# AberHu/TF-NAS

Measured on AMD Instinct MI355X. Metric: supernet search images/sec (w-step + alpha-step), higher is better.
Workload: dtype fp32

## Files before the change

### tf-nas_amd/csrc/gemm_core.h

```cpp
#pragma once
#include "tfnas_dev.h"

template <int NT>
struct GT {
    static constexpr int BM = 128, BK = 16, BN = 16 * NT;
    static constexpr int LDA = BM + 16;
    static constexpr int LDB = (BN % 32 == 16) ? BN : BN + 16;
    static constexpr int A_FLOATS = BK * LDA, B_FLOATS = BK * LDB;
    static constexpr int X3_FLOATS = 1584 * NT;
    static constexpr int LDS_FLOATS = 2 * (A_FLOATS + B_FLOATS) > X3_FLOATS ? 2 * (A_FLOATS + B_FLOATS) : X3_FLOATS;
    static constexpr int B_ITEMS = BN * 4;
    static constexpr int B_ITERS = (B_ITEMS + 255) / 256;
};

template <int NT>
__device__ __forceinline__ void acc_zero(f32x4 (&acc)[2][NT]) {
#pragma unroll
    for (int i = 0; i < 2; ++i)
#pragma unroll
        for (int j = 0; j < NT; ++j) acc[i][j] = zero4();
}

struct XfId {
    __device__ __forceinline__ f32x4 operator()(f32x4 v, int, int, int, int) const { return v; }
};

template <int NT, bool AK, bool BKC, bool BGUARD = true, class LA, class XA, class LB, class XB>
__device__ __forceinline__ void gemm_mainloop2(LA& la, XA& xa, LB& lb, XB& xb, int nchunks, f32x4 (&acc)[2][NT],
                                               float* lds) {
    using T = GT<NT>;
    using RA = decltype(la(0, 0, 0, 0));
    using RB = decltype(lb(0, 0, 0, 0));
    const int tid = threadIdx.x, lane = tid & 63, wrow = (tid >> 6) * 32;
    const int lr = lane & 15, lk = lane >> 4;
    RA ra[2];
    RB rb[T::B_ITERS];

#define TFNAS_A_IDX(i) const int idx = tid + 256 * (i), a0_ = AK ? (idx >> 2) : (idx >> 5), a1_ = AK ? (idx & 3) * 4 : (idx & 31) * 4
#define TFNAS_B_IDX(i)                                                      \
    const int idx = tid + 256 * (i), b0_ = BKC ? (idx >> 2) : idx / (T::BN / 4), \
              b1_ = BKC ? (idx & 3) * 4 : (idx % (T::BN / 4)) * 4
#define TFNAS_GLOAD(c)                                                                      \
    {                                                                                       \
        _Pragma("unroll") for (int i = 0; i < 2; ++i) {                                     \
            TFNAS_A_IDX(i);                                                                 \
            ra[i] = la((c), i, a0_, a1_);                                                      \
        }                                                                                   \
        _Pragma("unroll") for (int i = 0; i < T::B_ITERS; ++i) {                            \
            TFNAS_B_IDX(i);                                                                 \
            if (!BGUARD || idx < T::B_ITEMS) rb[i] = lb((c), i, b0_, b1_);                                \
        }                                                                                   \
    }
#define TFNAS_SSTORE(c, As, Bs)                                                             \
    {                                                                                       \
        _Pragma("unroll") for (int i = 0; i < 2; ++i) {                                     \
            TFNAS_A_IDX(i);                                                                 \
            const f32x4 v = xa(ra[i], (c), i, a0_, a1_);                                       \
            if (AK) {                                                                       \
                (As)[(a1_ + 0) * T::LDA + a0_] = v.x;                                       \
                (As)[(a1_ + 1) * T::LDA + a0_] = v.y;                                       \
                (As)[(a1_ + 2) * T::LDA + a0_] = v.z;                                       \
                (As)[(a1_ + 3) * T::LDA + a0_] = v.w;                                       \
            } else {                                                                        \
                st4(&(As)[a0_ * T::LDA + a1_], v);                                          \
            }                                                                               \
        }                                                                                   \
        _Pragma("unroll") for (int i = 0; i < T::B_ITERS; ++i) {                            \
            TFNAS_B_IDX(i);                                                                 \
            if (idx < T::B_ITEMS) {                                                         \
                const f32x4 v = xb(rb[i], (c), i, b0_, b1_);                                   \
                if (BKC) {                                                                  \
                    (Bs)[(b1_ + 0) * T::LDB + b0_] = v.x;                                   \
                    (Bs)[(b1_ + 1) * T::LDB + b0_] = v.y;                                   \
                    (Bs)[(b1_ + 2) * T::LDB + b0_] = v.z;                                   \
                    (Bs)[(b1_ + 3) * T::LDB + b0_] = v.w;                                   \
                } else {                                                                    \
                    st4(&(Bs)[b0_ * T::LDB + b1_], v);                                      \
                }                                                                           \
            }                                                                               \
        }                                                                                   \
    }

    float* As0 = lds;
    float* As1 = lds + T::A_FLOATS;
    float* Bs0 = lds + 2 * T::A_FLOATS;
    float* Bs1 = Bs0 + T::B_FLOATS;
#define TFNAS_MFMAS(As, Bs)                                                                 \
    _Pragma("unroll") for (int ks = 0; ks < 4; ++ks) {                                      \
        const int k = ks * 4 + lk;                                                          \
        const float a0 = (As)[k * T::LDA + wrow + lr];                                      \
        const float a1 = (As)[k * T::LDA + wrow + 16 + lr];                                 \
        _Pragma("unroll") for (int j = 0; j < NT; ++j) {                                    \
            const float b = (Bs)[k * T::LDB + 16 * j + lr];                                 \
            acc[0][j] = __builtin_amdgcn_mfma_f32_16x16x4f32(a0, b, acc[0][j], 0, 0, 0);    \
            acc[1][j] = __builtin_amdgcn_mfma_f32_16x16x4f32(a1, b, acc[1][j], 0, 0, 0);    \
        }                                                                                   \
    }

    if (nchunks > 0) {
        TFNAS_GLOAD(0);
        TFNAS_SSTORE(0, As0, Bs0);
    }
    __syncthreads();
    for (int c = 0; c < nchunks; ++c) {
        const bool more = (c + 1 < nchunks);
        if (more) TFNAS_GLOAD(c + 1);
        if (c & 1) { TFNAS_MFMAS(As1, Bs1); } else { TFNAS_MFMAS(As0, Bs0); }
        if (more) {
            if (c & 1) { TFNAS_SSTORE(c + 1, As0, Bs0); } else { TFNAS_SSTORE(c + 1, As1, Bs1); }
        }
        __syncthreads();
    }
#undef TFNAS_MFMAS
#undef TFNAS_GLOAD
#undef TFNAS_SSTORE
#undef TFNAS_A_IDX
#undef TFNAS_B_IDX
}

struct PreNone {
    __device__ __forceinline__ void operator()(int) const {}
};
template <int NT, bool BKC, class PRE, class LA, class XA, class LB, class XB>
__device__ __forceinline__ void gemm_mainloop_adirect(PRE& pre, LA& la, XA& xa, LB& lb, XB& xb, int nchunks,
                                                      f32x4 (&acc)[2][NT], float* lds) {
    using T = GT<NT>;
    using RA = decltype(la(0, 0, 0));
    using RB = decltype(lb(0, 0, 0));
    const int tid = threadIdx.x, lane = tid & 63;
    const int lr = lane & 15, lk = lane >> 4;
    RA ra[2];
    RB rb[T::B_ITERS];
    f32x4 cur[2];

#define TFNAS_B_IDX(i)                                                      \
    const int idx = tid + 256 * (i), b0_ = BKC ? (idx >> 2) : idx / (T::BN / 4), \
              b1_ = BKC ? (idx & 3) * 4 : (idx % (T::BN / 4)) * 4
#define TFNAS_GLOAD(c)                                                                      \
    {                                                                                       \
        pre(c);                                                                             \
        _Pragma("unroll") for (int i = 0; i < 2; ++i) ra[i] = la((c), i, 4 * lk);           \
        _Pragma("unroll") for (int i = 0; i < T::B_ITERS; ++i) {                            \
            TFNAS_B_IDX(i);                                                                 \
            if (idx < T::B_ITEMS) rb[i] = lb((c), b0_, b1_);                                \
        }                                                                                   \
    }
#define TFNAS_SSTORE(c, Bs)                                                                 \
    {                                                                                       \
        _Pragma("unroll") for (int i = 0; i < 2; ++i) cur[i] = xa(ra[i], (c), i, 4 * lk);   \
        _Pragma("unroll") for (int i = 0; i < T::B_ITERS; ++i) {                            \
            TFNAS_B_IDX(i);                                                                 \
            if (idx < T::B_ITEMS) {                                                         \
                const f32x4 v = xb(rb[i], (c), b0_, b1_);                                   \
                if (BKC) {                          \
                    const int r0_ = b1_ >> 2;                                               \
                    (Bs)[(r0_ + 0) * T::LDB + b0_] = v.x;                                   \
                    (Bs)[(r0_ + 4) * T::LDB + b0_] = v.y;                                   \
                    (Bs)[(r0_ + 8) * T::LDB + b0_] = v.z;                                   \
                    (Bs)[(r0_ + 12) * T::LDB + b0_] = v.w;                                  \
                } else {                                                                    \
                    st4(&(Bs)[((b0_ & 3) * 4 + (b0_ >> 2)) * T::LDB + b1_], v);             \
                }                                                                           \
            }                                                                               \
        }                                                                                   \
    }

    float* Bs0 = lds;
    float* Bs1 = lds + T::B_FLOATS;
    if (nchunks > 0) {
        TFNAS_GLOAD(0);
        TFNAS_SSTORE(0, Bs0);
    }
    __syncthreads();
    for (int c = 0; c < nchunks; ++c) {
        const float* Bs = (c & 1) ? Bs1 : Bs0;
        const bool more = (c + 1 < nchunks);
        if (more) TFNAS_GLOAD(c + 1);
#pragma unroll
        for (int ks = 0; ks < 4; ++ks) {
            const int k = ks * 4 + lk;
            const float a0 = cur[0][ks], a1 = cur[1][ks];
#pragma unroll
            for (int j = 0; j < NT; ++j) {
                const float b = Bs[k * T::LDB + 16 * j + lr];
                acc[0][j] = __builtin_amdgcn_mfma_f32_16x16x4f32(a0, b, acc[0][j], 0, 0, 0);
                acc[1][j] = __builtin_amdgcn_mfma_f32_16x16x4f32(a1, b, acc[1][j], 0, 0, 0);
            }
        }
        if (more) {
            if (c & 1) { TFNAS_SSTORE(c + 1, Bs0); } else { TFNAS_SSTORE(c + 1, Bs1); }
        }
        __syncthreads();
    }
#undef TFNAS_GLOAD
#undef TFNAS_SSTORE
#undef TFNAS_B_IDX
}

template <int NT, bool AK, bool BKC, class FA, class FB>
__device__ __forceinline__ void gemm_mainloop(FA& fa, FB& fb, int nchunks, f32x4 (&acc)[2][NT], float* lds) {
// ... 96 lines not shown
```

### tf-nas_amd/csrc/gemm_kernels.hip

```cpp
#include <stdlib.h>
#include <string.h>
#include "gemm_core.h"
#include "gemm_x3.h"
#include "kernels.h"
#include "prof.h"

__device__ __forceinline__ f32x4 stem_patch4(const float* __restrict__ img, const TfnasCellDesc& d, int p, int t0) {
    const int HW = d.H * d.W, n = p / HW, r = p - n * HW, ho = r / d.W, wo = r - ho * d.W;
    f32x4 v = zero4();
#pragma unroll
    for (int j = 0; j < 4; ++j) {
        const int t = t0 + j;
        if (t < 27) {
            const int ci = t / 9, rem = t - 9 * ci, ky = rem / 3, kx = rem - 3 * ky;
            const int hi = 2 * ho + ky - 1, wi = 2 * wo + kx - 1;
            if (hi >= 0 && hi < d.Hi && wi >= 0 && wi < d.Wi) v[j] = img[((size_t)(n * 3 + ci) * d.Hi + hi) * d.Wi + wi];
        }
    }
    return v;
}

constexpr int kLbBig = 3, kLbSmall = 4;
constexpr int kLbX3Big = 2, kLbX3Small = 3;
constexpr int gemm_lb(int nt, int mm) { return mm == 0 ? (nt >= 5 ? kLbBig : kLbSmall) : (nt >= 5 ? kLbX3Big : kLbX3Small); }
// ... 355 lines not shown
            const int o = min(c * 16 + kl, oc - 4);
            Raw2 r;
            r.a = ld4(drow[i] + o);
            r.b = ld4(qrow[i] + o);
            return r;
        };
        auto xa = [&](Raw2 r, int c, int i, int kl) -> f32x4 {
            const int o = c * 16 + kl;
            const f32x4 v = bn3_fold_dp(tab, min(o, oc - 4), r.a, r.b);
            return (rok[i] && o < oc) ? v : zero4();
        };
        auto lb = [&](int c, int kl, int n) -> f32x4 {
            const int o = c * 16 + kl;
            if (MM == 0 && !w_al) return (o < oc) ? ld4_guard(w + (size_t)o * mc, n0 + n, mc, false) : zero4();
            return ld4(w + (size_t)min(o, oc - 1) * mc + min(n0 + n, mc - 4));
        };
        auto xb = [&](f32x4 r, int c, int kl, int n) -> f32x4 {
            if (MM == 0 && !w_al) return r;
            return (c * 16 + kl < oc && n0 + n < mc) ? r : zero4();
        };
        PreNone pre;
        gemm_adirect<NT, false, MM>(pre, la, xa, lb, xb, nchunks, acc, lds);
        if (!FOLD) {
            emit_tile_rows<NT>(acc, lds, [&](int lrow, int lc, f32x4 v) {
                const int p = rt * 128 + lrow;
                if (p < Po && n0 + lc < mcp) st4_nt(dZ + ((size_t)p * M + off + n0 + lc), v);
            });
        } else {
            constexpr int LDC = T::BN + 4;
            const int w = tid >> 6, lane = tid & 63;
            const int pw0 = rt * 128 + w * 32;
            const int imgA = min(pw0, Po - 1) / HW, bnd = (imgA + 1) * HW;
            float sum[2][FOLD_Q][NC];
#pragma unroll
            for (int a = 0; a < 2; ++a)
#pragma unroll
                for (int q = 0; q < FOLD_Q; ++q)
#pragma unroll
                    for (int c = 0; c < NC; ++c) sum[a][q][c] = 0.f;
            const float* Dcol = D + off + n0;
            emit_tile_rows<NT>(acc, lds,
                               [&](int lrow, int lc, f32x4 v) {
                                   const int p = rt * 128 + lrow;
                                   if (p < Po && n0 + lc < mcp) st4_nt(dZ + ((size_t)p * M + off + n0 + lc), v);
                               },
                               [&](int i, const float* st) {
                                   if (d.act == TFNAS_ACT_RELU)
                                       fold_slab<NT, TFNAS_ACT_RELU>(st, LDC, Dcol, M, pw0 + 16 * i, Po, bnd, c2f, cokf, has_se, sum);
                                   else
                                       fold_slab<NT, TFNAS_ACT_SWISH>(st, LDC, Dcol, M, pw0 + 16 * i, Po, bnd, c2f, cokf, has_se, sum);
                               });
            static_assert(4 * 2 * FOLD_Q * T::BN + 4 <= T::LDS_FLOATS, "fold staging does not fit the GEMM LDS buffer");
            float* comb = lds;
            int* meta = reinterpret_cast<int*>(lds + 4 * 2 * FOLD_Q * T::BN);
#pragma unroll
            for (int a = 0; a < 2; ++a)
#pragma unroll
                for (int q = 0; q < FOLD_Q; ++q)
#pragma unroll
                    for (int c = 0; c < NC; ++c)
                        if (lane + 64 * c < T::BN) comb[((w * 2 + a) * FOLD_Q + q) * T::BN + lane + 64 * c] = sum[a][q][c];
            if (lane == 0) meta[w] = imgA;
            __syncthreads();
            const int img0 = min(rt * 128, Po - 1) / HW, imgL = min(rt * 128 + 127, Po - 1) / HW;
            const int nq = has_se ? FOLD_Q : 2;
            for (int o = tid; o < FOLD_SLOTS * FOLD_Q * T::BN; o += 256) {
                const int sl = o / (FOLD_Q * T::BN), q = (o / T::BN) % FOLD_Q, col = o % T::BN;
                if (img0 + sl > imgL || q >= nq || n0 + col >= mcp) continue;
                float t = 0.f;
#pragma unroll
                for (int ww = 0; ww < 4; ++ww)
#pragma unroll
                    for (int a = 0; a < 2; ++a)
                        if (meta[ww] + a - img0 == sl) t += comb[((ww * 2 + a) * FOLD_Q + q) * T::BN + col];
                rec[(((size_t)rt * FOLD_SLOTS + sl) * FOLD_Q + q) * M + off + n0 + col] = t;
            }
            __syncthreads();
        }
    }
}

constexpr int wgrad_lb(int nt) { return nt >= 5 ? 2 : (nt >= 3 ? 3 : 4); }

template <int NT, int ACT>
__global__ __launch_bounds__(256, wgrad_lb(NT)) void k_project_wgrad(TfnasCellDesc d, const float* __restrict__ dout,
                                                       const float* __restrict__ Pr, const float* __restrict__ D,
                                                       const float* __restrict__ gate,
                                                       const double* __restrict__ stats2,
                                                       const double* __restrict__ stats3,
                                                       const double* __restrict__ red3,
                                                       const float* __restrict__ wmix, int rows_per_split,
                                                       int ntiles_o, float* __restrict__ part, size_t out_size) {
    using T = GT<NT>;
    extern __shared__ __attribute__((aligned(16))) float lds[];
    const int g = blockIdx.z / ntiles_o, n0 = (blockIdx.z % ntiles_o) * T::BN;
    const int mc = d.g[g].mc, mcp = d.g[g].mcp, off = d.g[g].off;
    const bool has_se = d.g[g].se > 0;
    const float* gbase = has_se ? gate : D;
    const size_t se01 = has_se ? 1 : 0;
    size_t poff = 0;
    for (int gg = 0; gg < g; ++gg) poff += (size_t)d.g[gg].mc * d.oc;
    float* __restrict__ gw = part + (size_t)blockIdx.x * out_size + poff;
    const int m0 = blockIdx.y * 128;
    if (m0 >= mcp) return;
    const int HW = d.Ho * d.Wo, Po = d.N * HW, oc = d.oc, M = d.M;
    const int ocp = (oc + 15) & ~15;
    const int r0 = blockIdx.x * rows_per_split, r1 = min(Po, r0 + rows_per_split);
    const int nchunks = (r1 - r0 + 15) >> 4;
    const int tid = threadIdx.x, lane = tid & 63, lr = lane & 15, lq = lane >> 4, wrow = (tid >> 6) * 32;

    const Bn3Tab tab = bn3_tab_fill(lds + T::LDS_FLOATS, ocp, d, g, stats3, red3, wmix);
    const int mch = m0 + (tid & 31) * 4;
    const bool chok = mch < mcp;
    const size_t acol = (size_t)off + min(mch, mcp - 4);
    float2 c2[4];
#pragma unroll
    for (int j = 0; j < 4; ++j)
        c2[j] = (mch + j < mc) ? bn_consts(stats2 + 2 * (size_t)(off + mch + j), 1.0 / (double)Po, d.eps)
                               : make_float2(0.f, 0.f);
    __syncthreads();
    constexpr int BQ = T::BN / 4;
    int bcol[T::B_ITERS];
    bool bok[T::B_ITERS];
    f32x4 k_mean[T::B_ITERS], k_a3[T::B_ITERS], k_ab[T::B_ITERS], k_s[T::B_ITERS];
#pragma unroll
    for (int i = 0; i < T::B_ITERS; ++i) {
        const int idx = tid + 256 * i, o = n0 + (idx % BQ) * 4;
        bok[i] = idx < T::B_ITEMS && o < oc;
        bcol[i] = min(o, oc - 4);
#pragma unroll
        for (int j = 0; j < 4; ++j) {
            const int oo = bcol[i] + j;
            k_mean[i][j] = tab.mean[oo];
            k_a3[i][j] = tab.a3[oo];
            k_ab[i][j] = tab.a3[oo] * tab.b3[oo];
            k_s[i][j] = tab.rstd[oo] * tab.c3[oo] * tab.a3[oo];
        }
    }
    const float inv_hw = 1.f / (float)HW;
    const bool small_p = Po < (1 << 24);
    auto image_of = [&](int p) -> int {
        if (!small_p) return p / HW;
        int q = (int)((float)p * inv_hw);
        const int r = p - q * HW;
        q += (r >= HW) ? 1 : 0;
        q -= (r < 0) ? 1 : 0;
        return q;
    };

    f32x4 acc[2][NT];
    acc_zero<NT>(acc);
    auto la = [&](int c, int i, int kl, int m) -> Raw2 {
        const int p = min(r0 + c * 16 + kl, r1 - 1);
        Raw2 r;
        r.a = ld4(D + ((size_t)p * M + acol));
        r.b = ld4(gbase + ((size_t)image_of(p) * M + acol) * se01);
        return r;
    };
    auto xa = [&](Raw2 r, int c, int i, int kl, int m) -> f32x4 {
        f32x4 v = r.a;
#pragma unroll
        for (int j = 0; j < 4; ++j) v[j] = act_f<ACT>((v[j] - c2[j].x) * c2[j].y);
        if (has_se) v *= r.b;
        return (chok && r0 + c * 16 + kl < r1) ? v : zero4();
    };
    auto lb = [&](int c, int i, int kl, int n) -> Raw2 {
        const int p = min(r0 + c * 16 + kl, r1 - 1);
        Raw2 r;
        r.a = ld4(dout + (size_t)p * oc + bcol[i]);
        r.b = ld4(Pr + ((size_t)g * Po + p) * oc + bcol[i]);
        return r;
    };
    auto xb = [&](Raw2 r, int c, int i, int kl, int n) -> f32x4 {
        const f32x4 v = (k_a3[i] * r.a - k_ab[i]) - (r.b - k_mean[i]) * k_s[i];
        return (bok[i] && r0 + c * 16 + kl < r1) ? v : zero4();
    };
    gemm_mainloop2<NT, false, false, false>(la, xa, lb, xb, nchunks, acc, lds);
    const bool vec = (mc & 3) == 0;
#pragma unroll
    for (int i = 0; i < 2; ++i) {
        const int ch0 = m0 + wrow + 16 * i + 4 * lq;
#pragma unroll
        for (int j = 0; j < NT; ++j) {
            const int o = n0 + 16 * j + lr;
            if (o >= oc) continue;
            float* dst = gw + (size_t)o * mc + ch0;
            if (vec && ch0 + 3 < mc) {
                st4(dst, acc[i][j]);
            } else {
#pragma unroll
                for (int r = 0; r < 4; ++r)
                    if (ch0 + r < mc) dst[r] = acc[i][j][r];
            }
        }
    }
}

__device__ __forceinline__ f32x4 bn1_de(const f32x4* cb, f32x4 deh, f32x4 e) {
    f32x4 r;
#pragma unroll
    for (int j = 0; j < 4; ++j) {
        const f32x4 t = cb[j];
        const float eh = (e[j] - t.x) * t.y;
        r[j] = t.y * (deh[j] - t.z - eh * t.w);
    }
    return r;
}

__device__ __forceinline__ f32x4 sink_add(f32x4 v, float w, f32x4 g) {
    float px = w * g.x, py = w * g.y, pz = w * g.z, pw = w * g.w;
    asm volatile("" : "+v"(px), "+v"(py), "+v"(pz), "+v"(pw));
    f32x4 r;
    r.x = v.x + px; r.y = v.y + py; r.z = v.z + pz; r.w = v.w + pw;
    return r;
}

template <int NT, int MM>
__global__ __launch_bounds__(256, gemm_lb(NT, MM)) void k_expand_dgrad(TfnasCellDesc d, const float* __restrict__ dEh,
                                                      const float* __restrict__ x, const float* __restrict__ cb1,
                                                      const float* __restrict__ gram, const float* __restrict__ dout,
                                                      const float* __restrict__ wmix, float* __restrict__ dx,
                                                      float* __restrict__ dxp, int nsplit,
                                                      const float* __restrict__ add_src,
                                                      const float* __restrict__ add_scale, int xonly_slot = -1) {
    using T = GT<NT>;
    __shared__ __attribute__((aligned(16))) float lds[T::LDS_FLOATS];
    const int n0 = blockIdx.y * T::BN;
    const int P = d.N * d.H * d.W, ic = d.ic, M = d.M;
    const int nrt = (P + 127) >> 7;
    const int tid = threadIdx.x, lr = tid & 15, wrow = (tid >> 6) * 32;
    const int zs = (int)blockIdx.z;
    int mchunks = 0;
    for (int g = 0; g < d.G; ++g) mchunks += (d.g[g].mcp + 15) >> 4;
    const int nchunks_all = mchunks + ((ic + 15) >> 4);
    const bool xonly = xonly_slot >= 0;
    const int per = xonly ? nchunks_all - mchunks : (nchunks_all + nsplit - 1) / nsplit;
    const int cbeg = xonly ? mchunks : zs * per;
    const int nchunks = max(0, min(nchunks_all, cbeg + per) - cbeg);
    float* __restrict__ dst = xonly ? dxp + (size_t)xonly_slot * P * ic : (nsplit > 1 ? dxp + (size_t)blockIdx.z * P * ic : dx);
    const bool plain = nsplit == 1 && !xonly;
    const bool add_res = d.has_res && plain;
    const bool add_sink = add_src != nullptr && plain;
    const float sink_w = add_src ? add_scale[0] : 0.f;
    float sumw = 1.f;
    if (wmix) {
        sumw = 0.f;
        for (int g = 0; g < d.G; ++g) sumw += wmix[g];
    }

    for (int rt = blockIdx.x; rt < nrt; rt += gridDim.x) {
        f32x4 acc[2][NT];
        acc_zero<NT>(acc);
        bool is_x;
        int k0, klim_a, klim_b, ld_a;
        size_t aoff;
        const float* bsrc;
        const float* ssrc;
        auto pre = [&](int c) {
            c += cbeg;
            if (c >= mchunks) {
                is_x = true;
// ... 135 lines not shown
                for (int j = 0; j < NT; ++j) {
                    const int cc = n0 + 16 * j + lr;
                    if (cc < ic) out[(size_t)row * ic + cc] = acc[i][j][r];
                }
            }
        }
}

#ifndef GRAM1_MAX_K
#define GRAM1_MAX_K 1536
#endif
constexpr int GRAM1_GB = 8;
template <int GRAM1_NW>
__global__ __launch_bounds__(64 * GRAM1_NW) void k_gram1(TfnasCellDesc d, const float* __restrict__ cb1, float* __restrict__ gram) {
    __shared__ float part[GRAM1_NW][2][16][17];
    const int ic = d.ic;
    const int r0 = blockIdx.y * 16, c0 = blockIdx.x * 32;
    const int tid = threadIdx.x, wave = tid >> 6, lane = tid & 63, li = lane & 15, kq = lane >> 4;
    const f32x4* cb = reinterpret_cast<const f32x4*>(cb1);
    const int r = r0 + li, ca = c0 + li, cb_ = c0 + 16 + li;
    const bool row_w = r < ic, row_b = r == ic, oka = ca < ic, okb = cb_ < ic;
    const int ra = row_w ? r : 0, caa = oka ? ca : 0, cbb = okb ? cb_ : 0;
    f32x4 acc0 = zero4(), acc1 = zero4();
    int base = 0;
    for (int g = 0; g < d.G; ++g) {
        const float* __restrict__ W = d.g[g].w_expand;
        const int mc = d.g[g].mc, off = d.g[g].off;
        const int nstep = (mc + 3) >> 2, nbatch = (nstep + GRAM1_GB - 1) / GRAM1_GB;
        int b = (wave - base % GRAM1_NW + GRAM1_NW) % GRAM1_NW;
        for (; b < nbatch; b += GRAM1_NW) {
            const int s0 = b * GRAM1_GB;
            float a[GRAM1_GB], b0[GRAM1_GB], b1[GRAM1_GB];
            f32x4 t[GRAM1_GB];
#pragma unroll
            for (int u = 0; u < GRAM1_GB; ++u) {
                const int m = 4 * (s0 + u) + kq;
                const int mm = m < mc ? m : mc - 1;
                const float* wr = W + (size_t)mm * ic;
                t[u] = cb[off + mm];
                a[u] = wr[ra];
                b0[u] = wr[caa];
                b1[u] = wr[cbb];
            }
#pragma unroll
            for (int u = 0; u < GRAM1_GB; ++u) {
                const int m = 4 * (s0 + u) + kq;
                const bool okm = m < mc;
                const float sk = t[u].y * t[u].y * t[u].w;
                float av = row_w ? sk * a[u] : (row_b ? sk * t[u].x - t[u].y * t[u].z : 0.f);
                av = okm ? av : 0.f;
                const float bv0 = (okm && oka) ? b0[u] : 0.f, bv1 = (okm && okb) ? b1[u] : 0.f;
                acc0 = __builtin_amdgcn_mfma_f32_16x16x4f32(av, bv0, acc0, 0, 0, 0);
                acc1 = __builtin_amdgcn_mfma_f32_16x16x4f32(av, bv1, acc1, 0, 0, 0);
            }
        }
        base += nbatch;
    }
#pragma unroll
    for (int q = 0; q < 4; ++q) {
        part[wave][0][4 * kq + q][li] = acc0[q];
        part[wave][1][4 * kq + q][li] = acc1[q];
    }
    __syncthreads();
    for (int e = tid; e < 512; e += 64 * GRAM1_NW) {
        const int h = e >> 8, row = (e >> 4) & 15, col = e & 15;
        double v = 0.0;
#pragma unroll
        for (int w = 0; w < GRAM1_NW; ++w) v += (double)part[w][h][row][col];
        const int rr = r0 + row, cc = c0 + 16 * h + col;
        if (rr <= ic && cc < ic) gram[(size_t)rr * ic + cc] = (float)v;
    }
}

template <int NT, bool STEM, bool XG>
__global__ __launch_bounds__(256, wgrad_lb(NT)) void k_expand_wgrad(TfnasCellDesc d, const float* __restrict__ dEh,
                                                      const float* __restrict__ E, const float* __restrict__ cb1,
                                                      const float* __restrict__ x, int rows_per_split,
                                                      float* __restrict__ part, size_t out_size, size_t out_main) {
    using T = GT<NT>;
    __shared__ __attribute__((aligned(16))) float lds[T::LDS_FLOATS];
    const int ic = d.ic;
    int ty = blockIdx.y, g = 0;
    for (; g < d.G - 1; ++g) {
        const int t = (d.g[g].mcp + 127) >> 7;
        if (ty < t) break;
        ty -= t;
    }
    const int mc = d.g[g].mc, mcp = d.g[g].mcp, off = d.g[g].off;
    const bool last = XG && g == d.G - 1;
    size_t poff = 0;
    for (int gg = 0; gg < g; ++gg) poff += (size_t)d.g[gg].mc * ic;
    float* __restrict__ gw = part + (size_t)blockIdx.x * out_size + poff;
    float* __restrict__ gx = part + (size_t)blockIdx.x * out_size + out_main;
    const int m0 = ty * 128, n0 = blockIdx.z * T::BN;
    const int P = d.N * d.H * d.W, M = d.M;
    const int r0 = blockIdx.x * rows_per_split, r1 = min(P, r0 + rows_per_split);
    const int nchunks = (r1 - r0 + 15) >> 4;
    const int tid = threadIdx.x, lane = tid & 63, lr = lane & 15, lq = lane >> 4, wrow = (tid >> 6) * 32;

    const int mch = m0 + (tid & 31) * 4;
    const bool chok = mch < mcp;
    const size_t acol = (size_t)off + min(mch, mcp - 4);
    f32x4 k_mu = zero4(), k_r = zero4(), k_rt1 = zero4(), k_s = zero4();
    if (!XG) {
#pragma unroll
        for (int j = 0; j < 4; ++j) {
            const f32x4 t = (mch + j < mcp) ? reinterpret_cast<const f32x4*>(cb1)[off + mch + j] : zero4();
            k_mu[j] = t.x;
            k_r[j] = t.y;
            k_rt1[j] = t.y * t.z;
            k_s[j] = t.y * t.y * t.w;
        }
    }
    const int ext = mch - mcp;
    const bool ax = last && ext >= 0 && ext < ic, aone = last && ext == ic;
    const float* __restrict__ abase = ax ? x + ext : dEh + acol;
    const size_t apitch = ax ? (size_t)ic : (size_t)M;
    const bool aok = chok || ax;
    constexpr int BQ = T::BN / 4;
    int bcol[T::B_ITERS];
    bool bok[T::B_ITERS];
#pragma unroll
    for (int i = 0; i < T::B_ITERS; ++i) {
        const int idx = tid + 256 * i, cc = n0 + (idx % BQ) * 4;
        bok[i] = idx < T::B_ITEMS && cc < ic;
        bcol[i] = STEM ? cc : min(cc, ic - 4);
    }

    f32x4 acc[2][NT];
    acc_zero<NT>(acc);
    auto la = [&](int c, int i, int kl, int m) -> Raw2 {
        const int p = min(r0 + c * 16 + kl, r1 - 1);
        Raw2 r;
        if (XG) {
            r.a = ld4(abase + (size_t)p * apitch);
            r.b = r.a;
        } else {
            const size_t at = (size_t)p * M + acol;
            r.a = ld4(dEh + at);
            r.b = ld4(E + at);
        }
        return r;
    };
    auto xa = [&](Raw2 r, int c, int i, int kl, int m) -> f32x4 {
        if (XG) {
            f32x4 v = aok ? r.a : zero4();
            if (aone) v.x = 1.f;
            return (r0 + c * 16 + kl < r1) ? v : zero4();
        }
        const f32x4 v = (k_r * r.a - k_rt1) - (r.b - k_mu) * k_s;
        return (chok && r0 + c * 16 + kl < r1) ? v : zero4();
    };
    auto lb = [&](int c, int i, int kl, int n) -> f32x4 {
        if (STEM) {
            const int p = r0 + c * 16 + kl;
            return (p < r1 && bok[i]) ? stem_patch4(x, d, p, bcol[i]) : zero4();
        }
        const int p = min(r0 + c * 16 + kl, r1 - 1);
        return ld4(x + (size_t)p * ic + bcol[i]);
    };
    auto xb = [&](f32x4 r, int c, int i, int kl, int n) -> f32x4 {
        if (STEM) return r;
        return (bok[i] && r0 + c * 16 + kl < r1) ? r : zero4();
    };
    gemm_mainloop2<NT, false, false, false>(la, xa, lb, xb, nchunks, acc, lds);
#pragma unroll
    for (int i = 0; i < 2; ++i)
#pragma unroll
        for (int r = 0; r < 4; ++r) {
            const int ch = m0 + wrow + 16 * i + 4 * lq + r;
            float* __restrict__ row = nullptr;
            if (ch < mc) row = gw + (size_t)ch * ic;
            else if (last && ch >= mcp && ch - mcp <= ic) row = gx + (size_t)(ch - mcp) * ic;
            if (row) {
#pragma unroll
                for (int j = 0; j < NT; ++j) {
                    const int cc = n0 + 16 * j + lr;
                    if (cc < ic) row[cc] = acc[i][j][r];
                }
            }
        }
}

__global__ __launch_bounds__(256) void k_expand_wgrad_fix(TfnasCellDesc d, const float* __restrict__ cb1,
                                                          const double* __restrict__ red, size_t out_main) {
    __shared__ double ps[4][64];
    const int ic = d.ic, lane = threadIdx.x & 63, wv = threadIdx.x >> 6;
    const size_t e = (size_t)blockIdx.x * 64 + lane;
    const bool ok = e < out_main;
    int g = 0;
    size_t poff = 0;
    for (; g < d.G - 1; ++g) {
        const size_t n = (size_t)d.g[g].mc * ic;
        if (e < poff + n) break;
        poff += n;
    }
    const int m = ok ? (int)((e - poff) / ic) : 0, c = ok ? (int)(e - poff - (size_t)m * ic) : 0;
    const double* __restrict__ Gx = red + out_main;
    const float* __restrict__ w = d.g[g].w_expand + (size_t)m * ic;
    double wg0 = 0.0, wg1 = 0.0;
    for (int k = 4 * wv; k < ic; k += 16) {
        const f32x4 wq = ld4(w + k);
        wg0 += (double)wq.x * Gx[(size_t)k * ic + c] + (double)wq.z * Gx[(size_t)(k + 2) * ic + c];
        wg1 += (double)wq.y * Gx[(size_t)(k + 1) * ic + c] + (double)wq.w * Gx[(size_t)(k + 3) * ic + c];
    }
    ps[wv][lane] = wg0 + wg1;
    __syncthreads();
    if (wv == 0 && ok) {
        const double wg = (ps[0][lane] + ps[1][lane]) + (ps[2][lane] + ps[3][lane]);
        const f32x4 t = reinterpret_cast<const f32x4*>(cb1)[d.g[g].off + m];
        const double sx = Gx[(size_t)ic * ic + c], mu = t.x, r = t.y, t1 = t.z, t2 = t.w;
        const float v = (float)(r * (red[e] - t1 * sx - t2 * r * (wg - mu * sx)));
        float* __restrict__ o = d.g[g].g_expand + (e - poff);
        *o = (d.flags & TFNAS_CELL_ACCUM_WGRAD) ? *o + v : v;
    }
}

static const int kNtSmall[] = {1, 2, 3, 4, 5, 7};
static constexpr int kGtLdsFloats[8] = {0, GT<1>::LDS_FLOATS, GT<2>::LDS_FLOATS, GT<3>::LDS_FLOATS, GT<4>::LDS_FLOATS,
                                        GT<5>::LDS_FLOATS, 0, GT<7>::LDS_FLOATS};

#define NT_CASE(n, ...) case n: { constexpr int NT = n; __VA_ARGS__; } break;
#define DISPATCH_NT_GROUPS(nt, ...)   \
    switch (nt) {                     \
        NT_CASE(4, __VA_ARGS__)       \
        NT_CASE(5, __VA_ARGS__)       \
        NT_CASE(7, __VA_ARGS__)       \
        default: return TFNAS_EINVAL; \
    }
#define DISPATCH_NT(nt, ...)                         \
    switch (nt) {                                    \
        NT_CASE(1, __VA_ARGS__)                      \
        NT_CASE(2, __VA_ARGS__)                      \
        NT_CASE(3, __VA_ARGS__)                      \
        default: DISPATCH_NT_GROUPS(nt, __VA_ARGS__) \
    }
#define DISPATCH_MM(mode, ...)                                 \
    switch (mode) {                                            \
        case 0: { constexpr int MM = 0; __VA_ARGS__; } break;  \
        case 1: { constexpr int MM = 1; __VA_ARGS__; } break;  \
        case 3: { constexpr int MM = 3; __VA_ARGS__; } break;  \
        default: { constexpr int MM = 6; __VA_ARGS__; } break; \
    }
#define DISPATCH_ACT(act, ...)                                                        \
    if ((act) == TFNAS_ACT_RELU) { constexpr int ACT = TFNAS_ACT_RELU; __VA_ARGS__; } \
    else { constexpr int ACT = TFNAS_ACT_SWISH; __VA_ARGS__; }

static int g_gemm_mode = 6;
int gemm_mode() { return g_gemm_mode & 7; }
int set_gemm_mode(int m) {
    const int base = m & ~TFNAS_GEMM_EVERYWHERE;
    if (base != 0 && base != 1 && base != 3 && base != 6) return TFNAS_EINVAL;
    g_gemm_mode = m;
    return 0;
}
static inline int gemm_word(const TfnasCellDesc& d) { return (d.gemm_mode & TFNAS_GEMM_EXPLICIT) ? d.gemm_mode : g_gemm_mode; }
int gemm_mode_of(const TfnasCellDesc& d) { return gemm_word(d) & 7; }
static int gemm_arith(const TfnasCellDesc& d, bool dgrad) {
    for (int g = 0; g < d.G; ++g)
        if (d.g[g].mc & 3) return 0;
    const int m = gemm_mode_of(d);
    if (!dgrad || m == 0 || (gemm_word(d) & TFNAS_GEMM_EVERYWHERE)) return m;
    if (m == 1) return m;
    return (d.G > 1 && d.Ho * d.Wo <= 196) ? m : 0;
}
static inline int gemm_slots(int nt, int mm) { return 256 * gemm_lb(nt, mm); }

static size_t stats_row_cap(size_t row_floats) {
    const size_t fit = TFNAS_PART_FLOATS / (row_floats ? row_floats : 1);
    return fit < 1024 ? fit : 1024;
}

static int row_blocks(int rows, int other_blocks, size_t cap, int slots, int max_gx = 1024) {
    const int nrt = cdiv(rows, 128);
    const int other = other_blocks > 0 ? other_blocks : 1;
    int lim = nrt;
    if ((size_t)lim > cap) lim = (int)cap;
    if (lim > max_gx) lim = max_gx;
    if (lim < 1) lim = 1;
    long best_cost = -1;
    int best = 1;
    for (int gx = 1; gx <= lim; ++gx) {
        const long cost = (long)cdiv(gx * other, slots) * cdiv(nrt, gx);
        if (best_cost < 0 || cost <= best_cost) {
            best_cost = cost;
            best = gx;
        }
    }
    return best;
}

static int pick_nt_groups(const TfnasCellDesc& d) {
    int min_mcp = 1 << 30;
    for (int g = 0; g < d.G; ++g) min_mcp = d.g[g].mcp < min_mcp ? d.g[g].mcp : min_mcp;
    if (min_mcp >= 200) return 4;
    static const int cands[] = {4, 5, 7};
    int best = 4;
    long best_pad = -1;
    for (int i = 0; i < 3; ++i) {
        long pad = 0;
        for (int g = 0; g < d.G; ++g) pad += (long)cdiv(d.g[g].mcp, 16 * cands[i]) * 16 * cands[i];
        if (best_pad < 0 || pad < best_pad || (pad == best_pad && cands[i] > best)) {
            best_pad = pad;
            best = cands[i];
        }
    }
    return best;
}
static int group_tiles(const TfnasCellDesc& d, int width, int last_extra = 0) {
    int t = 0;
    for (int g = 0; g < d.G; ++g) t += cdiv(d.g[g].mcp + (g == d.G - 1 ? last_extra : 0), width);
// ... 11 lines not shown
}
static GemmPlan plan_cols(int n) {
    GemmPlan p{};
    p.nt = pick_nt(n, kNtSmall, 6);
    p.tiles = cdiv(n, 16 * p.nt);
    return p;
}

GemmPlan gemm_plan_expand_fwd(const TfnasCellDesc& d) {
    GemmPlan p{};
    p.var = d.mode == TFNAS_MODE_STEM ? GEMM_STEM : GEMM_PLAIN;
    p.nt = p.var == GEMM_STEM ? (d.g[0].mcp <= 32 ? 2 : 4) : pick_nt_groups(d);
    p.mm = gemm_arith(d, false);
    p.tiles = group_tiles(d, 16 * p.nt);
    p.grid = dim3(row_blocks(d.N * d.H * d.W, p.tiles, stats_row_cap(2 * (size_t)d.M), gemm_slots(p.nt, p.mm)), p.tiles);
    return p;
}

int launch_expand_fwd(const TfnasCellDesc& d, const float* x, float* E, double* stats1, float* part,
                      hipStream_t s) {
    ProfScope _prof(TK_EXPAND_FWD, s);
    const GemmPlan p = gemm_plan_expand_fwd(d);
    DISPATCH_MM(p.mm, {
        if (p.var == GEMM_STEM)
            hipLaunchKernelGGL((p.nt == 2 ? k_expand_fwd<2, true, MM> : k_expand_fwd<4, true, MM>), p.grid, dim3(256), 0, s, d, x, E, part);
        else
            DISPATCH_NT_GROUPS(p.nt, { hipLaunchKernelGGL((k_expand_fwd<NT, false, MM>), p.grid, dim3(256), 0, s, d, x, E, part); })
    })
    _prof.stop();
    return launch_reduce_rows(part, p.grid.x, 2 * d.M, 2 * (size_t)d.M, stats1, nullptr, s);
}

#ifndef TFNAS_WSPLIT_DGRAD
#define TFNAS_WSPLIT_DGRAD 2
#endif
#ifndef TFNAS_WSPLIT_PFWD
#define TFNAS_WSPLIT_PFWD 2
#endif
GemmPlan gemm_plan_project_fwd(const TfnasCellDesc& d) {
    GemmPlan p = plan_cols(d.oc);
    p.mm = gemm_arith(d, false);
    const int mcp_max = max_mcp(d), ncols2 = 2 * d.G * d.oc;
    const int Po = d.N * d.Ho * d.Wo, nrt = cdiv(Po, 128);
    p.shm = (kGtLdsFloats[p.nt] + 2 * ((mcp_max + 15) & ~15)) * sizeof(float);
    int nsplit = 1;
    const int wgs = nrt * p.tiles * d.G, kch = cdiv(mcp_max, 16);
    if (wgs < 512 && kch >= 16 && (d.oc & 3) == 0 && d.oc <= 1024) {
        nsplit = cdiv(1024, wgs);
        if (nsplit > 4) nsplit = 4;
        if (nsplit > kch / 8) nsplit = kch / 8;
        if (d.need_wgrad && d.G == 1 && nsplit > TFNAS_WSPLIT_PFWD) nsplit = TFNAS_WSPLIT_PFWD;
        const size_t per = (size_t)d.G * Po * d.oc, rows2 = 256 * (size_t)ncols2;
        while (nsplit > 1 && (nsplit - 1) * per + rows2 > TFNAS_PART_FLOATS) --nsplit;
    }
    p.splits = nsplit;
    p.parts = nsplit - 1;
    if (p.parts) p.grid = dim3(nrt, p.tiles, d.G * nsplit);
    else p.grid = dim3(row_blocks(Po, p.tiles * d.G, stats_row_cap((size_t)ncols2), gemm_slots(p.nt, p.mm)), p.tiles, d.G);
    int gx2 = cdiv(Po, 64);
    if (gx2 > 256) gx2 = 256;
    p.rps = cdiv(Po, gx2);
    p.grid2 = dim3(cdiv(Po, p.rps), d.G);
    return p;
}

int launch_project_fwd(const TfnasCellDesc& d, const float* D, const float* gate, const double* stats2,
                       float* Pr, double* stats3, float* part, hipStream_t s) {
    ProfScope _prof(TK_PROJECT_FWD, s);
    const GemmPlan p = gemm_plan_project_fwd(d);
    const int ncols2 = 2 * d.G * d.oc, Po = d.N * d.Ho * d.Wo;
    float* prp = p.parts ? part : nullptr;
    float* rows = part + (size_t)p.parts * d.G * Po * d.oc;
    DISPATCH_MM(p.mm, DISPATCH_NT(p.nt, DISPATCH_ACT(d.act, {
        hipLaunchKernelGGL((k_project_fwd<NT, ACT, MM>), p.grid, dim3(256), p.shm, s, d, D, gate, stats2, Pr, part, p.splits, prp);
    })))
    if (p.parts) hipLaunchKernelGGL(k_pr_reduce, p.grid2, dim3(256), 0, s, Pr, prp, p.parts, d.G, Po, d.oc, p.rps, rows);
    _prof.stop();
    return launch_reduce_rows(rows, p.parts ? p.grid2.x : p.grid.x, ncols2, (size_t)ncols2, stats3, nullptr, s);
}

GemmPlan gemm_plan_project_dgrad(const TfnasCellDesc& d, bool fold) {
    GemmPlan p{};
    p.var = fold ? GEMM_FOLD : GEMM_PLAIN;
    p.nt = pick_nt_groups(d);
    p.mm = gemm_arith(d, true);
    p.tiles = group_tiles(d, 16 * p.nt);
    p.grid = dim3(row_blocks(d.N * d.Ho * d.Wo, p.tiles, 1u << 30, gemm_slots(p.nt, p.mm)), p.tiles);
    p.shm = (kGtLdsFloats[p.nt] + 4 * ((d.oc + 15) & ~15)) * sizeof(float);
    return p;
}

int launch_project_dgrad(const TfnasCellDesc& d, const float* dout, const float* Pr, const double* stats3,
                         const double* red3, const float* wmix, float* dZ, hipStream_t s, const float* D,
                         const double* stats2, float* rec) {
    ProfScope _prof(TK_PROJECT_DGRAD, s);
    if (rec && (!D || !stats2)) return TFNAS_ENULL;
    const GemmPlan p = gemm_plan_project_dgrad(d, rec != nullptr);
    DISPATCH_MM(p.mm, DISPATCH_NT_GROUPS(p.nt, {
        if (p.var == GEMM_FOLD)
            hipLaunchKernelGGL((k_project_dgrad<NT, MM, true>), p.grid, dim3(256), p.shm, s, d, dout, Pr, stats3, red3, wmix, dZ,
                               D, stats2, rec);
        else
            hipLaunchKernelGGL((k_project_dgrad<NT, MM>), p.grid, dim3(256), p.shm, s, d, dout, Pr, stats3, red3, wmix, dZ);
    }))
    return (int)hipGetLastError();
}

static void plan_row_splits(GemmPlan& p, int rows, int mtiles, int ztiles, size_t scratch) {
    const int target = 256 * wgrad_lb(p.nt), min_rows = 128, out_tiles = mtiles * ztiles;
    int splits = target / (out_tiles > 0 ? out_tiles : 1);
    const size_t cap = scratch / (p.out > 0 ? p.out : 1);
    if ((size_t)splits > cap) splits = (int)cap;
    if (splits < 1) splits = 1;
    int rps = cdiv(rows, splits);
    if (rps < min_rows) rps = min_rows;
    p.rps = ((rps + 15) / 16) * 16;
    p.splits = cdiv(rows, p.rps);
    p.grid = dim3(p.splits, mtiles, ztiles);
}
static int reduce_group_wgrads(const TfnasCellDesc& d, const GemmPlan& p, const float* part, int n, float* TfnasGroup::*dst,
                               hipStream_t s) {
    size_t poff = 0;
    for (int g = 0; g < d.G; ++g) {
        const int cols = d.g[g].mc * n;
        int rc = launch_reduce_rows(part + poff, p.splits, cols, p.out, nullptr, d.g[g].*dst, s, wgrad_accum(d));
        if (rc) return rc;
        poff += cols;
    }
    return (int)hipGetLastError();
}

GemmPlan gemm_plan_project_wgrad(const TfnasCellDesc& d) {
    GemmPlan p = plan_cols(d.oc);
    p.out = mid_floats(d, d.oc);
    plan_row_splits(p, d.N * d.Ho * d.Wo, cdiv(max_mcp(d), 128), p.tiles * d.G, TFNAS_PART_FLOATS);
    p.shm = (kGtLdsFloats[p.nt] + 5 * ((d.oc + 15) & ~15)) * sizeof(float);
    return p;
}

int launch_project_wgrad(const TfnasCellDesc& d, const float* dout, const float* Pr, const float* D,
                         const float* gate, const double* stats2, const double* stats3, const double* red3,
                         const float* wmix, float* part, hipStream_t s) {
    ProfScope _prof(TK_PROJECT_WGRAD, s);
    const GemmPlan p = gemm_plan_project_wgrad(d);
    DISPATCH_NT(p.nt, DISPATCH_ACT(d.act, {
        hipLaunchKernelGGL((k_project_wgrad<NT, ACT>), p.grid, dim3(256), p.shm, s, d, dout, Pr, D, gate, stats2,
                           stats3, red3, wmix, p.rps, p.tiles, part, p.out);
    }))
    _prof.stop();
    return reduce_group_wgrads(d, p, part, d.oc, &TfnasGroup::g_proj, s);
}

size_t expand_gram_floats(const TfnasCellDesc& d) { return (size_t)(d.ic + 4) * d.ic; }
static int mid_chunks(const TfnasCellDesc& d) { return group_tiles(d, 16); }

GemmPlan gemm_plan_expand_gram(const TfnasCellDesc& d, size_t scratch_floats) {
    GemmPlan p{};
    if (!(d.route & TFNAS_ROUTE_GRAM2) && mid_floats(d, 1) <= GRAM1_MAX_K) {
        p.var = GEMM_GRAM1;
        p.grid = dim3(cdiv(d.ic, 32), cdiv(d.ic + 1, 16));
        return p;
    }
    p = plan_cols(d.ic);
    const size_t gsz = expand_gram_floats(d);
    const int mchunks = mid_chunks(d), mtiles = cdiv(d.ic + 1, 128);
    int splits = cdiv(512, mtiles * p.tiles);
    if (splits > mchunks / 4) splits = mchunks / 4;
    if ((size_t)splits > scratch_floats / gsz) splits = (int)(scratch_floats / gsz);
    if (splits < 1) splits = 1;
    p.rps = cdiv(mchunks, splits);
    p.splits = cdiv(mchunks, p.rps);
    p.grid = dim3(p.splits, mtiles, p.tiles);
    return p;
}

int launch_expand_gram(const TfnasCellDesc& d, const float* cb1, float* scratch, size_t scratch_floats, float* gram,
                       hipStream_t s) {
    ProfScope _prof(TK_SMALL, s);
    const GemmPlan p = gemm_plan_expand_gram(d, scratch_floats);
    if (p.var == GEMM_GRAM1) {
        for (int g = 0; g < d.G; ++g)
            if (d.g[g].mc < 1) return TFNAS_EINVAL;
        if (d.mode == TFNAS_MODE_HEAD) hipLaunchKernelGGL(k_gram1<16>, p.grid, dim3(1024), 0, s, d, cb1, gram);
        else hipLaunchKernelGGL(k_gram1<4>, p.grid, dim3(256), 0, s, d, cb1, gram);
        return (int)hipGetLastError();
    }
    const size_t gsz = expand_gram_floats(d);
    if (scratch_floats < gsz) return TFNAS_ERANGE;
    DISPATCH_NT(p.nt, { hipLaunchKernelGGL(k_expand_gram<NT>, p.grid, dim3(256), 0, s, d, cb1, p.rps, p.splits, scratch); })
    _prof.stop();
    return launch_reduce_rows(scratch, p.splits, (int)gsz, gsz, nullptr, gram, s);
}

GemmPlan gemm_plan_expand_dgrad(const TfnasCellDesc& d, bool split, int nsl) {
    GemmPlan p = plan_cols(d.ic);
    p.mm = gemm_arith(d, true);
    const int P = d.N * d.H * d.W, out_tiles = cdiv(P, 128) * p.tiles;
    p.splits = 1;
    if (split && nsl < 0 && out_tiles < 512) {
        const int mchunks = mid_chunks(d);
        int ns = cdiv(1024, out_tiles);
        if (ns > 16) ns = 16;
        if (ns > mchunks / 4) ns = mchunks / 4;
        if (d.need_wgrad && d.G == 1 && ns > TFNAS_WSPLIT_DGRAD) ns = TFNAS_WSPLIT_DGRAD;
        p.splits = ns < 1 ? 1 : ns;
    }
    p.grid = dim3(row_blocks(P, p.tiles * p.splits, 1u << 30, gemm_slots(p.nt, p.mm), 4096), p.tiles, p.splits);
    p.parts = nsl >= 0 ? nsl + 1 : (p.splits > 1 ? p.splits : 0);
    size_t blocks = cdiv64((size_t)P * d.ic / 4, 256 * 2);
    p.grid2 = dim3((unsigned)(blocks > 2048 ? 2048 : blocks));
    return p;
}

int launch_expand_dgrad(const TfnasCellDesc& d, const float* dEh, const float* x, const float* cb1, const float* gram,
                        const float* dout, const float* wmix, float* dx, float* dxp, hipStream_t s,
                        const float* add_src, const float* add_scale, int nsl) {
    const GemmPlan p = gemm_plan_expand_dgrad(d, dxp != nullptr, nsl);
    {
        ProfScope _prof(TK_EXPAND_DGRAD, s);
        DISPATCH_MM(p.mm, DISPATCH_NT(p.nt, {
            hipLaunchKernelGGL((k_expand_dgrad<NT, MM>), p.grid, dim3(256), 0, s, d, dEh, x, cb1, gram, dout, wmix, dx, dxp, p.splits,
                               add_src, add_scale, nsl);
        }))
    }
    if (p.parts) {
        ProfScope _p2(TK_SMALL, s);
        hipLaunchKernelGGL(k_dx_reduce, p.grid2, dim3(256), 0, s, d, dxp, p.parts, gram, dout, wmix, dx, add_src, add_scale);
    }
    return (int)hipGetLastError();
}

static size_t xg_red_floats(const GemmPlan& p) { return p.var == GEMM_XG ? 2 * p.out + 4 : 0; }

GemmPlan gemm_plan_expand_wgrad(const TfnasCellDesc& d) {
    GemmPlan p = plan_cols(d.ic);
    const int P = d.N * d.H * d.W;
    if (d.mode == TFNAS_MODE_STEM) p.var = GEMM_STEM;
    else if (!(d.route & TFNAS_ROUTE_XG_OFF) && (d.ic & 3) == 0 &&
             ((d.route & TFNAS_ROUTE_XG_ALL) || (size_t)P * d.M * sizeof(float) >= ((size_t)100 << 20)))
        p.var = GEMM_XG;
    const int next = p.var == GEMM_XG ? d.ic + 1 : 0;
    p.out_main = mid_floats(d, d.ic);
    p.out = p.out_main + (size_t)next * d.ic;
    plan_row_splits(p, P, group_tiles(d, 128, next), p.tiles, TFNAS_PART_FLOATS - xg_red_floats(p));
    return p;
}

int launch_expand_wgrad(const TfnasCellDesc& d, const float* dEh, const float* E, const float* cb1,
                        const float* x, float* part, hipStream_t s) {
    ProfScope _prof(TK_EXPAND_WGRAD, s);
    const GemmPlan p = gemm_plan_expand_wgrad(d);
    const size_t red_floats = xg_red_floats(p);
    if (p.var != GEMM_XG && !E) return TFNAS_ENULL;
    if (red_floats + p.out > TFNAS_PART_FLOATS) return TFNAS_ERANGE;
    if (p.var == GEMM_STEM && p.nt != 2) return TFNAS_EINVAL;
    DISPATCH_NT(p.nt, {
        auto k = p.var == GEMM_XG ? k_expand_wgrad<NT, false, true> : k_expand_wgrad<NT, false, false>;
        if (p.var == GEMM_STEM) k = k_expand_wgrad<2, true, false>;
        hipLaunchKernelGGL(k, p.grid, dim3(256), 0, s, d, dEh, E, cb1, x, p.rps, part, p.out, p.out_main);
    })
    _prof.stop();
    if (p.var != GEMM_XG) return reduce_group_wgrads(d, p, part, d.ic, &TfnasGroup::g_expand, s);
    double* red = reinterpret_cast<double*>((uintptr_t)(part + TFNAS_PART_FLOATS - red_floats + 3) & ~(uintptr_t)15);
    int rc = launch_reduce_rows(part, p.splits, (int)p.out, p.out, red, nullptr, s);
    if (rc) return rc;
    ProfScope _p2(TK_EXPAND_WGRAD, s);
    hipLaunchKernelGGL(k_expand_wgrad_fix, dim3((unsigned)cdiv64(p.out_main, 64)), dim3(256), 0, s, d, cb1, red, p.out_main);
    return (int)hipGetLastError();
}
```

Before: 3890.

## Split K across waves for short M tiles in weight-gradient GEMMs

When a weight-gradient tile covers only 32 or 64 channel rows, the otherwise idle waves now take a share of the K dimension instead of computing padding. Their partial accumulators are then folded through LDS into the owning waves. Only the owning waves write results. The project dgrad also forces NT=2 for stem cells with small channel counts. This targets wasted MFMA work on narrow groups, at the cost of extra LDS traffic, extra barriers and some divergence.

```diff
diff --git a/tf-nas_amd/csrc/gemm_core.h b/tf-nas_amd/csrc/gemm_core.h
--- a/tf-nas_amd/csrc/gemm_core.h
+++ b/tf-nas_amd/csrc/gemm_core.h
@@ -25,26 +25,33 @@
     __device__ __forceinline__ f32x4 operator()(f32x4 v, int, int, int, int) const { return v; }
 };
 
-template <int NT, bool AK, bool BKC, bool BGUARD = true, class LA, class XA, class LB, class XB>
+template <int NT, bool AK, bool BKC, bool BGUARD = true, int WM = 4, class LA, class XA, class LB, class XB>
 __device__ __forceinline__ void gemm_mainloop2(LA& la, XA& xa, LB& lb, XB& xb, int nchunks, f32x4 (&acc)[2][NT],
                                                float* lds) {
     using T = GT<NT>;
     using RA = decltype(la(0, 0, 0, 0));
     using RB = decltype(lb(0, 0, 0, 0));
-    const int tid = threadIdx.x, lane = tid & 63, wrow = (tid >> 6) * 32;
+    static_assert(WM == 4 || (!AK && (WM == 1 || WM == 2)), "short tiles: M-contiguous A, 32 or 64 rows");
+    constexpr int A_ITERS = WM == 4 ? 2 : 1, AQ = 8 * WM, KW = 4 / WM;
+    const int tid = threadIdx.x, lane = tid & 63;
+    const int wv = WM == 4 ? (tid >> 6) : __builtin_amdgcn_readfirstlane(tid >> 6);
+    const int wrow = (WM == 4 ? wv : wv % WM) * 32, ksub = WM == 4 ? 0 : wv / WM;
+    const bool astage = WM >= 2 || wv < 2;
     const int lr = lane & 15, lk = lane >> 4;
-    RA ra[2];
+    RA ra[A_ITERS];
     RB rb[T::B_ITERS];
 
-#define TFNAS_A_IDX(i) const int idx = tid + 256 * (i), a0_ = AK ? (idx >> 2) : (idx >> 5), a1_ = AK ? (idx & 3) * 4 : (idx & 31) * 4
+#define TFNAS_A_IDX(i) const int idx = tid + 256 * (i), a0_ = AK ? (idx >> 2) : (idx / AQ), a1_ = AK ? (idx & 3) * 4 : (idx % AQ) * 4
 #define TFNAS_B_IDX(i)                                                      \
     const int idx = tid + 256 * (i), b0_ = BKC ? (idx >> 2) : idx / (T::BN / 4), \
               b1_ = BKC ? (idx & 3) * 4 : (idx % (T::BN / 4)) * 4
 #define TFNAS_GLOAD(c)                                                                      \
     {                                                                                       \
-        _Pragma("unroll") for (int i = 0; i < 2; ++i) {                                     \
-            TFNAS_A_IDX(i);                                                                 \
-            ra[i] = la((c), i, a0_, a1_);                                                      \
+        if (astage) {                                                                       \
+            _Pragma("unroll") for (int i = 0; i < A_ITERS; ++i) {                           \
+                TFNAS_A_IDX(i);                                                             \
+                ra[i] = la((c), i, a0_, a1_);                                               \
+            }                                                                               \
         }                                                                                   \
         _Pragma("unroll") for (int i = 0; i < T::B_ITERS; ++i) {                            \
             TFNAS_B_IDX(i);                                                                 \
@@ -53,7 +60,8 @@
     }
 #define TFNAS_SSTORE(c, As, Bs)                                                             \
     {                                                                                       \
-        _Pragma("unroll") for (int i = 0; i < 2; ++i) {                                     \
+        _Pragma("unroll") for (int i = 0; i < A_ITERS; ++i) {                               \
+            if (!astage) break;                                                             \
             TFNAS_A_IDX(i);                                                                 \
             const f32x4 v = xa(ra[i], (c), i, a0_, a1_);                                       \
             if (AK) {                                                                       \
@@ -86,8 +94,8 @@
     float* Bs0 = lds + 2 * T::A_FLOATS;
     float* Bs1 = Bs0 + T::B_FLOATS;
 #define TFNAS_MFMAS(As, Bs)                                                                 \
-    _Pragma("unroll") for (int ks = 0; ks < 4; ++ks) {                                      \
-        const int k = ks * 4 + lk;                                                          \
+    _Pragma("unroll") for (int ks = 0; ks < WM; ++ks) {                                     \
+        const int k = (ks * KW + ksub) * 4 + lk;                                            \
         const float a0 = (As)[k * T::LDA + wrow + lr];                                      \
         const float a1 = (As)[k * T::LDA + wrow + 16 + lr];                                 \
         _Pragma("unroll") for (int j = 0; j < NT; ++j) {                                    \
@@ -116,6 +124,42 @@
 #undef TFNAS_SSTORE
 #undef TFNAS_A_IDX
 #undef TFNAS_B_IDX
+}
+
+__host__ __device__ __forceinline__ int wgrad_tiles(int rows) { return (rows + 127) >> 7; }
+__host__ __device__ __forceinline__ int wgrad_tile(int rows, int t, int& m0) {
+    m0 = t * 128;
+    const int left = rows - m0;
+    return left > 64 ? 4 : (left > 32 ? 2 : 1);
+}
+
+template <int NT>
+__device__ __forceinline__ void wgrad_fold_ksplit(f32x4 (&acc)[2][NT], float* lds, int wm) {
+    static_assert(3 * 256 * NT <= GT<NT>::LDS_FLOATS, "k-split staging does not fit the GEMM LDS buffer");
+    if (wm == 4) return;
+    const int lane = threadIdx.x & 63, w = threadIdx.x >> 6;
+    const int slab = w & (wm - 1), share = wm == 2 ? (w >> 1) : w, shares = 4 / wm;
+#pragma unroll
+    for (int i = 0; i < 2; ++i) {
+        if (share > 0) {
+            float* st = lds + ((share - 1) * wm + slab) * 256 * NT + lane;
+#pragma unroll
+            for (int j = 0; j < NT; ++j)
+#pragma unroll
+                for (int r = 0; r < 4; ++r) st[(j * 4 + r) * 64] = acc[i][j][r];
+        }
+        __syncthreads();
+        if (share == 0) {
+            for (int q = 1; q < shares; ++q) {
+                const float* st = lds + ((q - 1) * wm + slab) * 256 * NT + lane;
+#pragma unroll
+                for (int j = 0; j < NT; ++j)
+#pragma unroll
+                    for (int r = 0; r < 4; ++r) acc[i][j][r] += st[(j * 4 + r) * 64];
+            }
+        }
+        __syncthreads();
+    }
 }
 
 struct PreNone {
diff --git a/tf-nas_amd/csrc/gemm_kernels.hip b/tf-nas_amd/csrc/gemm_kernels.hip
--- a/tf-nas_amd/csrc/gemm_kernels.hip
+++ b/tf-nas_amd/csrc/gemm_kernels.hip
@@ -461,6 +461,12 @@
 
 constexpr int wgrad_lb(int nt) { return nt >= 5 ? 2 : (nt >= 3 ? 3 : 4); }
 
+#define WGRAD_MAINLOOP(wm)                                                                           \
+    if ((wm) == 4) gemm_mainloop2<NT, false, false, false, 4>(la, xa, lb, xb, nchunks, acc, lds);     \
+    else if ((wm) == 2) gemm_mainloop2<NT, false, false, false, 2>(la, xa, lb, xb, nchunks, acc, lds); \
+    else gemm_mainloop2<NT, false, false, false, 1>(la, xa, lb, xb, nchunks, acc, lds);               \
+    wgrad_fold_ksplit<NT>(acc, lds, (wm))
+
 template <int NT, int ACT>
 __global__ __launch_bounds__(256, wgrad_lb(NT)) void k_project_wgrad(TfnasCellDesc d, const float* __restrict__ dout,
                                                        const float* __restrict__ Pr, const float* __restrict__ D,
@@ -480,8 +486,9 @@
     size_t poff = 0;
     for (int gg = 0; gg < g; ++gg) poff += (size_t)d.g[gg].mc * d.oc;
     float* __restrict__ gw = part + (size_t)blockIdx.x * out_size + poff;
-    const int m0 = blockIdx.y * 128;
-    if (m0 >= mcp) return;
+    if ((int)blockIdx.y >= wgrad_tiles(mcp)) return;
+    int m0;
+    const int wm = wgrad_tile(mcp, blockIdx.y, m0);
     const int HW = d.Ho * d.Wo, Po = d.N * HW, oc = d.oc, M = d.M;
     const int ocp = (oc + 15) & ~15;
     const int r0 = blockIdx.x * rows_per_split, r1 = min(Po, r0 + rows_per_split);
@@ -489,7 +496,7 @@
     const int tid = threadIdx.x, lane = tid & 63, lr = lane & 15, lq = lane >> 4, wrow = (tid >> 6) * 32;
 
     const Bn3Tab tab = bn3_tab_fill(lds + T::LDS_FLOATS, ocp, d, g, stats3, red3, wmix);
-    const int mch = m0 + (tid & 31) * 4;
+    const int mch = m0 + (tid & (8 * wm - 1)) * 4;
     const bool chok = mch < mcp;
     const size_t acol = (size_t)off + min(mch, mcp - 4);
     float2 c2[4];
@@ -554,8 +561,9 @@
         const f32x4 v = (k_a3[i] * r.a - k_ab[i]) - (r.b - k_mean[i]) * k_s[i];
         return (bok[i] && r0 + c * 16 + kl < r1) ? v : zero4();
     };
-    gemm_mainloop2<NT, false, false, false>(la, xa, lb, xb, nchunks, acc, lds);
+    WGRAD_MAINLOOP(wm);
     const bool vec = (mc & 3) == 0;
+    if ((tid >> 6) >= wm) return;
 #pragma unroll
     for (int i = 0; i < 2; ++i) {
         const int ch0 = m0 + wrow + 16 * i + 4 * lq;
@@ -857,23 +865,25 @@
     const int ic = d.ic;
     int ty = blockIdx.y, g = 0;
     for (; g < d.G - 1; ++g) {
-        const int t = (d.g[g].mcp + 127) >> 7;
+        const int t = wgrad_tiles(d.g[g].mcp);
         if (ty < t) break;
         ty -= t;
     }
     const int mc = d.g[g].mc, mcp = d.g[g].mcp, off = d.g[g].off;
     const bool last = XG && g == d.G - 1;
+    int m0;
+    const int wm = wgrad_tile(mcp + (last ? ic + 1 : 0), ty, m0);
     size_t poff = 0;
     for (int gg = 0; gg < g; ++gg) poff += (size_t)d.g[gg].mc * ic;
     float* __restrict__ gw = part + (size_t)blockIdx.x * out_size + poff;
     float* __restrict__ gx = part + (size_t)blockIdx.x * out_size + out_main;
-    const int m0 = ty * 128, n0 = blockIdx.z * T::BN;
+    const int n0 = blockIdx.z * T::BN;
     const int P = d.N * d.H * d.W, M = d.M;
     const int r0 = blockIdx.x * rows_per_split, r1 = min(P, r0 + rows_per_split);
     const int nchunks = (r1 - r0 + 15) >> 4;
     const int tid = threadIdx.x, lane = tid & 63, lr = lane & 15, lq = lane >> 4, wrow = (tid >> 6) * 32;
 
-    const int mch = m0 + (tid & 31) * 4;
+    const int mch = m0 + (tid & (8 * wm - 1)) * 4;
     const bool chok = mch < mcp;
     const size_t acol = (size_t)off + min(mch, mcp - 4);
     f32x4 k_mu = zero4(), k_r = zero4(), k_rt1 = zero4(), k_s = zero4();
@@ -938,7 +948,8 @@
         if (STEM) return r;
         return (bok[i] && r0 + c * 16 + kl < r1) ? r : zero4();
     };
-    gemm_mainloop2<NT, false, false, false>(la, xa, lb, xb, nchunks, acc, lds);
+    WGRAD_MAINLOOP(wm);
+    if ((tid >> 6) >= wm) return;
 #pragma unroll
     for (int i = 0; i < 2; ++i)
 #pragma unroll
@@ -1002,6 +1013,11 @@
         NT_CASE(5, __VA_ARGS__)       \
         NT_CASE(7, __VA_ARGS__)       \
         default: return TFNAS_EINVAL; \
+    }
+#define DISPATCH_NT_GROUPS_STEM(nt, ...)  \
+    switch (nt) {                                                        \
+        NT_CASE(2, __VA_ARGS__)                                          \
+        default: DISPATCH_NT_GROUPS(nt, __VA_ARGS__)                     \
     }
 #define DISPATCH_NT(nt, ...)                         \
     switch (nt) {                                    \
@@ -1179,7 +1195,7 @@
 GemmPlan gemm_plan_project_dgrad(const TfnasCellDesc& d, bool fold) {
     GemmPlan p{};
     p.var = fold ? GEMM_FOLD : GEMM_PLAIN;
-    p.nt = pick_nt_groups(d);
+    p.nt = (d.mode == TFNAS_MODE_STEM && max_mcp(d) <= 32) ? 2 : pick_nt_groups(d);
     p.mm = gemm_arith(d, true);
     p.tiles = group_tiles(d, 16 * p.nt);
     p.grid = dim3(row_blocks(d.N * d.Ho * d.Wo, p.tiles, 1u << 30, gemm_slots(p.nt, p.mm)), p.tiles);
@@ -1193,7 +1209,7 @@
     ProfScope _prof(TK_PROJECT_DGRAD, s);
     if (rec && (!D || !stats2)) return TFNAS_ENULL;
     const GemmPlan p = gemm_plan_project_dgrad(d, rec != nullptr);
-    DISPATCH_MM(p.mm, DISPATCH_NT_GROUPS(p.nt, {
+    DISPATCH_MM(p.mm, DISPATCH_NT_GROUPS_STEM(p.nt, {
         if (p.var == GEMM_FOLD)
             hipLaunchKernelGGL((k_project_dgrad<NT, MM, true>), p.grid, dim3(256), p.shm, s, d, dout, Pr, stats3, red3, wmix, dZ,
                                D, stats2, rec);
@@ -1230,7 +1246,7 @@
 GemmPlan gemm_plan_project_wgrad(const TfnasCellDesc& d) {
     GemmPlan p = plan_cols(d.oc);
     p.out = mid_floats(d, d.oc);
-    plan_row_splits(p, d.N * d.Ho * d.Wo, cdiv(max_mcp(d), 128), p.tiles * d.G, TFNAS_PART_FLOATS);
+    plan_row_splits(p, d.N * d.Ho * d.Wo, wgrad_tiles(max_mcp(d)), p.tiles * d.G, TFNAS_PART_FLOATS);
     p.shm = (kGtLdsFloats[p.nt] + 5 * ((d.oc + 15) & ~15)) * sizeof(float);
     return p;
 }
@@ -1339,7 +1355,9 @@
     const int next = p.var == GEMM_XG ? d.ic + 1 : 0;
     p.out_main = mid_floats(d, d.ic);
     p.out = p.out_main + (size_t)next * d.ic;
-    plan_row_splits(p, P, group_tiles(d, 128, next), p.tiles, TFNAS_PART_FLOATS - xg_red_floats(p));
+    int mtiles = 0;
+    for (int g = 0; g < d.G; ++g) mtiles += wgrad_tiles(d.g[g].mcp + (g == d.G - 1 ? next : 0));
+    plan_row_splits(p, P, mtiles, p.tiles, TFNAS_PART_FLOATS - xg_red_floats(p));
     return p;
 }
 
```

Result: no change. 3892 (median of 2 runs) (+0.1%).
